# KyanChen/RSPrompter

Hardware: AMD Instinct MI355X
Metric: images/sec (1024x1024 synthetic tiles, rsprompter_anchor SAM-ViT-H, full predict path) (higher is better)
Workload: dtype f32 (fp32 in/out; GEMMs and attention as fp16x3 split-precision MFMA with fp32 accumulate); 1 GPU; rsprompter_anchor SAM-ViT-huge, batch 8x1024x1024 per GPU, 10 classes, seeded synthetic weights (the per-GPU slice of BASELINE.json configs[3] on 1 GPU); parallelism=single GPU

## Files before the change

### rsprompter_amd/csrc/t2i_fold.hip

```cpp
#include <type_traits>
#include "rsp_common.h"

namespace {

typedef __attribute__((address_space(3))) void* lptr_f;
typedef short v4s_f __attribute__((ext_vector_type(4)));

constexpr int FKT = 32, FNW = 3, FNT = FNW * 64, FNBUF = 2;
constexpr int FD = 256;
constexpr int FKCPR = 36, FPCPR = 17;
constexpr int FK_UNITS = FKT * FKCPR;
constexpr int FP_UNITS = 576;
constexpr int FTILE_UNITS = 2 * FK_UNITS + 2 * FP_UNITS;
constexpr int FNDMA = FTILE_UNITS / FNT;
constexpr int FBUF_BYTES = FTILE_UNITS * 16;
constexpr float F_PSCALE_LOG2 = 14.0f;
constexpr unsigned F_OOB = 0x80000000u;

static_assert(FK_UNITS % FNT == 0 && FP_UNITS % FNT == 0, "every DMA instruction reads one plane");

template <int I, int N, class F>
__device__ __forceinline__ void static_for_f(F&& f) {
  if constexpr (I < N) {
    f(std::integral_constant<int, I>{});
    static_for_f<I + 1, N>(f);
  }
}

__device__ __forceinline__ void split8_fast_f(const float* x, half8_t& hi, half8_t& lo) {
  float m1 = -1.0f;
  asm volatile("" : "+v"(m1));
#pragma unroll
  for (int i = 0; i < 8; i += 2) {
    const half2_t h2 = __builtin_bit_cast(half2_t, __builtin_amdgcn_cvt_pkrtz(x[i], x[i + 1]));
    const float r0 = __builtin_fmaf((float)h2[0], m1, x[i]), r1 = __builtin_fmaf((float)h2[1], m1, x[i + 1]);
    const half2_t l2 = __builtin_bit_cast(half2_t, __builtin_amdgcn_cvt_pkrtz(r0, r1));
    hi[i] = h2[0]; hi[i + 1] = h2[1]; lo[i] = l2[0]; lo[i + 1] = l2[1];
  }
}

struct T2iFoldP {
  const half_t* khi; const half_t* klo; int64_t k_rows;
  const half_t* phi; const half_t* plo;
  const half_t* qhi; const half_t* qlo; int64_t q_rows;
  const half_t* thi; const half_t* tlo;
  float* u;
  int N, ncols;
  float c_main, c_pe;
  float u_unscale;
};

template <int NPE>
__global__ __launch_bounds__(FNT) void sam_t2i_fold_kernel(const T2iFoldP p) {
  __shared__ __attribute__((aligned(1024))) unsigned char smem[FNBUF][FBUF_BYTES];
  __shared__ __attribute__((aligned(1024))) unsigned char sQl[FNW * 16 * 1024];
  const int tid = threadIdx.x, lane = tid & 63;
  const int wave = __builtin_amdgcn_readfirstlane(tid >> 6);
  const int hh = lane >> 5, l31 = lane & 31;
  const int r = blockIdx.x;
  const int N = p.N;
  const int nt = N / FKT;

  const __amdgpu_buffer_rsrc_t rKh = __builtin_amdgcn_make_buffer_rsrc(const_cast<half_t*>(p.khi), 0, (int)(p.k_rows * 512), 0x00020000);
  const __amdgpu_buffer_rsrc_t rKl = __builtin_amdgcn_make_buffer_rsrc(const_cast<half_t*>(p.klo), 0, (int)(p.k_rows * 512), 0x00020000);
  const __amdgpu_buffer_rsrc_t rPh = __builtin_amdgcn_make_buffer_rsrc(const_cast<half_t*>(p.phi), 0, N * 256, 0x00020000);
  const __amdgpu_buffer_rsrc_t rPl = __builtin_amdgcn_make_buffer_rsrc(const_cast<half_t*>(p.plo), 0, N * 256, 0x00020000);
  unsigned voff_k[6], voff_p[3];
#pragma unroll
  for (int i = 0; i < 6; ++i) {
    const int v = i * FNT + tid;
    const int row = v / FKCPR, pc = v - row * FKCPR;
    const int c = pc ^ ((row >> 2) & 3);
    voff_k[i] = pc < 32 ? (unsigned)(((int64_t)(c >> 2) * p.k_rows + row) * 64 + (c & 3) * 16) : F_OOB;
  }
#pragma unroll
  for (int i = 0; i < 3; ++i) {
    const int v = i * FNT + tid;
    const int row = v / FPCPR, pc = v - row * FPCPR;
    voff_p[i] = (row < FKT && pc < 16) ? (unsigned)(((int64_t)(pc >> 2) * N + row) * 64 + (pc & 3) * 16) : F_OOB;
  }
  const unsigned so_k0 = (unsigned)((int64_t)r * N * 64);
  const rsp_lds_addr_t smem_a = rsp_lds_addr((lptr_f)&smem[0][0]);
  auto issue_slot = [&](auto ic, int kt, int buf) {
    constexpr int i = decltype(ic)::value;
    const unsigned so_k = so_k0 + (unsigned)kt * (FKT * 64), so_p = (unsigned)kt * (FKT * 64);
    const rsp_lds_addr_t l = smem_a + buf * FBUF_BYTES + (i * FNT + wave * 64) * 16;
    const __amdgpu_buffer_rsrc_t rs = i < 6 ? rKh : (i < 12 ? rKl : (i < 15 ? rPh : rPl));
    const unsigned vo = i < 12 ? voff_k[i < 12 ? i % 6 : 0] : voff_p[i >= 12 ? (i - 12) % 3 : 0];
    const unsigned so = i < 12 ? so_k : so_p;
    RSP_BUFFER_LOAD_LDS_B128(rs, l, vo, so);
  };
  static_for_f<0, FNDMA>([&](auto ic) { issue_slot(ic, 0, 0); });

  const int64_t qrow = (int64_t)r * 96 + wave * 32 + l31;
  const int hb = NPE == 8 ? 0 : min((wave * 32) / (p.ncols >> 3), 8 - NPE);
  half8_t qh[16], th[NPE], tl[NPE];
  unsigned char* const my_ql = sQl + wave * (16 * 1024) + lane * 16;
#pragma unroll
  for (int st = 0; st < 16; ++st) {
    const int64_t o = ((int64_t)(st >> 1) * p.q_rows + qrow) * 32 + 16 * (st & 1) + 8 * hh;
    qh[st] = *reinterpret_cast<const half8_t*>(p.qhi + o);
    *reinterpret_cast<half8_t*>(my_ql + st * 1024) = *reinterpret_cast<const half8_t*>(p.qlo + o);
  }
#pragma unroll
  for (int s_ = 0; s_ < NPE; ++s_) {
    const int st = hb + s_;
    const int64_t o = ((int64_t)(st >> 1) * p.q_rows + qrow) * 32 + 16 * (st & 1) + 8 * hh;
    th[s_] = *reinterpret_cast<const half8_t*>(p.thi + o);
    tl[s_] = *reinterpret_cast<const half8_t*>(p.tlo + o);
  }

  f32x16 acc_o[8];
#pragma unroll
  for (int db = 0; db < 8; ++db)
#pragma unroll
    for (int e = 0; e < 16; ++e) acc_o[db][e] = 0.f;
  float m_run = -INFINITY, l_run = 0.f;

  const int k_row_off = l31 * (FKCPR * 16);
  const int k_swz = (l31 >> 2) & 3;
  const int p_row_off = l31 * (FPCPR * 16);
  const int li = lane & 15, g16 = (lane >> 4) & 1;
  const int v_row = 4 * hh + (li >> 2);
  const int v_c = 2 * g16 + ((li & 3) >> 1);
  const int v_b = 8 * (li & 1);

  for (int kt = 0; kt < nt; ++kt) {
    const int buf = kt & 1;
    asm volatile("s_waitcnt vmcnt(0)" ::: "memory");
    __builtin_amdgcn_s_barrier();
    const bool has_next = kt + 1 < nt;
    if (has_next) static_for_f<0, FNDMA>([&](auto ic) { issue_slot(ic, kt + 1, buf ^ 1); });
    const unsigned char* sb = &smem[buf][0];
    const unsigned char* sK0 = sb;
    const unsigned char* sK1 = sb + FK_UNITS * 16;
    const unsigned char* sP0 = sb + 2 * FK_UNITS * 16;
    const unsigned char* sP1 = sP0 + FP_UNITS * 16;

    f32x16 s0, s1, sp;
#pragma unroll
    for (int e = 0; e < 16; ++e) { s0[e] = 0.f; s1[e] = 0.f; sp[e] = 0.f; }
    {
      constexpr int LA = 1, NB = LA + 1;
      half8_t kfh[NB], kfl[NB];
      auto kread = [&](int st, half8_t& h8, half8_t& l8) {
        const int off = k_row_off + (((2 * st + hh) ^ k_swz) << 4);
        h8 = *reinterpret_cast<const half8_t*>(sK0 + off);
        l8 = *reinterpret_cast<const half8_t*>(sK1 + off);
      };
      auto pread = [&](int s_, half8_t& h8, half8_t& l8) {
        const int off = p_row_off + ((2 * (hb + s_) + hh) << 4);
        h8 = *reinterpret_cast<const half8_t*>(sP0 + off);
        l8 = *reinterpret_cast<const half8_t*>(sP1 + off);
      };
      half8_t qlf[NB];
      auto fetch = [&](auto jc) {
        constexpr int j = decltype(jc)::value, sl = j % NB;
        if constexpr (j < 16) {
          kread(j, kfh[sl], kfl[sl]);
          qlf[sl] = *reinterpret_cast<const half8_t*>(my_ql + j * 1024);
        } else if constexpr (j < 16 + NPE) pread(j - 16, kfh[sl], kfl[sl]);
      };
      static_for_f<0, LA>([&](auto jc) { fetch(jc); });
      static_for_f<0, 16 + NPE>([&](auto ic) {
        constexpr int i = decltype(ic)::value, cur = i % NB;
// ... 85 lines not shown
    for (int db = 0; db < 8; ++db)
#pragma unroll
      for (int g = 0; g < 4; ++g) {
        f32x4 o;
#pragma unroll
        for (int c = 0; c < 4; ++c) o[c] = acc_o[db][4 * g + c] * inv;
        *reinterpret_cast<f32x4*>(dst + db * 32 + 8 * g + 4 * hh) = o;
      }
  }
}

}

extern "C" int rsp_sam_t2i_fold(const uint16_t* keys_hi, const uint16_t* keys_lo, int64_t k_rows, int32_t keys_e,
                                const uint16_t* pek_hi, const uint16_t* pek_lo, int32_t pek_e, const uint16_t* qp_hi,
                                const uint16_t* qp_lo, int32_t qp_e, const uint16_t* tqx_hi, const uint16_t* tqx_lo,
                                int32_t tqx_e, int64_t q_rows, float* u, int32_t R, int32_t N, int32_t ncols,
                                rsp_stream_t stream) {
  if (!keys_hi || !keys_lo || !pek_hi || !pek_lo || !qp_hi || !qp_lo || !tqx_hi || !tqx_lo || !u || R < 0 || N <= 0 ||
      (N % FKT) || ncols <= 0 || ncols > 96 || (ncols & 7) || k_rows < (int64_t)R * N || q_rows < (int64_t)R * 96 ||
      k_rows * 512 > 0x7fffffffLL || (int64_t)N * 256 > 0x7fffffffLL)
    return RSP_EINVAL;
  if (R == 0) return RSP_OK;
  T2iFoldP p;
  p.khi = reinterpret_cast<const half_t*>(keys_hi); p.klo = reinterpret_cast<const half_t*>(keys_lo); p.k_rows = k_rows;
  p.phi = reinterpret_cast<const half_t*>(pek_hi); p.plo = reinterpret_cast<const half_t*>(pek_lo);
  p.qhi = reinterpret_cast<const half_t*>(qp_hi); p.qlo = reinterpret_cast<const half_t*>(qp_lo); p.q_rows = q_rows;
  p.thi = reinterpret_cast<const half_t*>(tqx_hi); p.tlo = reinterpret_cast<const half_t*>(tqx_lo);
  p.u = u; p.N = N; p.ncols = ncols;
  constexpr float LOG2E_F = 1.4426950408889634f;
  p.c_main = ldexpf(1.0f, -(keys_e + qp_e)) * LOG2E_F;
  p.c_pe = ldexpf(1.0f, -(pek_e + tqx_e)) * LOG2E_F;
  p.u_unscale = ldexpf(1.0f, -keys_e);
  const bool five = ncols >= 56;
  const dim3 g(R), b(FNT);
  hipStream_t s = (hipStream_t)stream;
  if (five) hipLaunchKernelGGL((sam_t2i_fold_kernel<5>), g, b, 0, s, p);
  else hipLaunchKernelGGL((sam_t2i_fold_kernel<8>), g, b, 0, s, p);
  RSP_CHECK_LAUNCH();
  return RSP_OK;
}
```

### rsprompter_amd/sam_decoder.py

```python
import math

import numpy as np
import torch

from . import ops
from .nnutil import HIPModule, add_param, infer_sam_arch, nchw_view, nhwc_view
from .registry import MODELS

HID = 256
HEADS = 8
MLP_DIM = 2048
N_MASK_TOKENS = 4


def _upscale2_k_order():
    return [32 * ((kp >> 4) >> 1) + 8 * ((8 * ((kp >> 4) & 1) + (kp & 7)) >> 2) + 4 * ((kp >> 3) & 1) + (kp & 3) for kp in range(64)]


def _add_linear(root, name, cout, cin):
    add_param(root, name + '.weight', (cout, cin))
    add_param(root, name + '.bias', (cout,))


def _add_ln(root, name, c):
# ... 13 lines not shown
    return root


HOOK_FORMS = ('accepted forms: attention_similarity 4-D [1 | B * Pb, 1, 1, N] (one bias row over the N image positions, shared '
              'or per prompt set; no per-head, per-token or other shape), with at most ops.SAM_T2I_MAX_TOKENS = 12 tokens; '
              'target_embedding [..., 256] that broadcasts to [B, Pb, 1, 256] (every other dimension 1 or equal)')


def persam_hooks(attention_similarity, target_embedding, B, Pb, N, T):
    R = B * Pb
    bias = te = None
    if attention_similarity is not None:
        a = attention_similarity
        if not torch.is_tensor(a) or a.dim() != 4 or a.shape[1] != 1 or a.shape[2] != 1 or a.shape[3] != N or \
                a.shape[0] not in (1, R):
            raise NotImplementedError(f'attention_similarity of shape {tuple(getattr(a, "shape", ()))} for B * Pb = {R}, N = {N}; '
                                      + HOOK_FORMS)
        if T > ops.SAM_T2I_MAX_TOKENS:
            raise NotImplementedError(f'attention_similarity with {T} tokens (the generic attention takes no bias); ' + HOOK_FORMS)
        bias = a.reshape(a.shape[0], N).to(torch.float32).contiguous()
    if target_embedding is not None:
        t = target_embedding
        ok = torch.is_tensor(t) and 1 <= t.dim() <= 4 and t.shape[-1] == HID
        if ok:
            b, pb, tk = ((1, 1, 1) + tuple(t.shape[:-1]))[-3:]
            ok = b in (1, B) and pb in (1, Pb) and tk == 1
        if not ok:
            raise NotImplementedError(f'target_embedding of shape {tuple(getattr(t, "shape", ()))} for B = {B}, Pb = {Pb}; '
                                      + HOOK_FORMS)
        t = t.to(torch.float32).reshape(b, pb, HID)
        te = t.reshape(1, HID) if b * pb == 1 else t.expand(B, Pb, HID).reshape(R, HID)
        te = te.contiguous()
    return bias, te


class SamMaskDecoderHIP(HIPModule):

    def __init__(self):
        super().__init__()
        add_param(self, 'iou_token.weight', (1, HID))
        add_param(self, 'mask_tokens.weight', (N_MASK_TOKENS, HID))
        for i in range(2):
            p = f'transformer.layers.{i}'
            _add_attn(self, p + '.self_attn', HID)
            _add_attn(self, p + '.cross_attn_token_to_image', HID // 2)
            _add_attn(self, p + '.cross_attn_image_to_token', HID // 2)
            for j in range(1, 5):
                _add_ln(self, f'{p}.layer_norm{j}', HID)
            _add_linear(self, p + '.mlp.lin1', MLP_DIM, HID)
            _add_linear(self, p + '.mlp.lin2', HID, MLP_DIM)
        _add_attn(self, 'transformer.final_attn_token_to_image', HID // 2)
        _add_ln(self, 'transformer.layer_norm_final_attn', HID)
        add_param(self, 'upscale_conv1.weight', (HID, HID // 4, 2, 2))
        add_param(self, 'upscale_conv1.bias', (HID // 4,))
        add_param(self, 'upscale_conv2.weight', (HID // 4, HID // 8, 2, 2))
        add_param(self, 'upscale_conv2.bias', (HID // 8,))
        _add_ln(self, 'upscale_layer_norm', HID // 4)
        for i in range(N_MASK_TOKENS):
            p = f'output_hypernetworks_mlps.{i}'
            _add_linear(self, p + '.proj_in', HID, HID)
            _add_linear(self, p + '.layers.0', HID, HID)
            _add_linear(self, p + '.proj_out', HID // 8, HID)
        _add_linear(self, 'iou_prediction_head.proj_in', HID, HID)
        _add_linear(self, 'iou_prediction_head.layers.0', HID, HID)
        _add_linear(self, 'iou_prediction_head.proj_out', N_MASK_TOKENS, HID)
        self._pe_cache = {}
# ... 50 lines not shown
                t[name] = ops.gemm(pe_rows, P[name])
            for pre, p in (('0.cross_attn_token_to_image', 'transformer.layers.0.cross_attn_token_to_image'),
                           ('1.cross_attn_token_to_image', 'transformer.layers.1.cross_attn_token_to_image'),
                           ('final', 'transformer.final_attn_token_to_image')):
                vb = _g(self, p + '.v_proj').bias
                t[pre + '.kv_proj'] = torch.cat([t[pre + '.k_proj'], vb.unsqueeze(0).expand(pe_rows.shape[0], -1)],
                                                1).contiguous()
                t[pre + '.pek_planes'] = ops.to_planes(t[pre + '.k_proj'])
            t['_table'] = pe_rows
            self._pe_cache = {key: t}
        return self._pe_cache[key]

    @staticmethod
    def _pe_key(pe_rows):
        return (pe_rows.data_ptr(), tuple(pe_rows.shape), pe_rows._version)

    def _ln(self, x, name, eps=1e-6, planes=False):
        m = _g(self, name)
        return ops.layernorm(x, m.weight, m.bias, eps, planes=planes)

    def _t2i(self, tq, kv, ao, R, T, N, kv_map=None, bias=None):
        d2, dh2 = HID // 2, (HID // 2) // HEADS
        if bias is not None:
            if T > ops.SAM_T2I_MAX_TOKENS:
                raise NotImplementedError(f'attention_similarity with {T} tokens; ' + HOOK_FORMS)
            return ops.sam_t2i_attention_bias(tq, kv, bias, ao, R=R, T=T, N=N, scale=dh2 ** -0.5, kv_map=kv_map)
        if T <= ops.SAM_T2I_MAX_TOKENS:
            return ops.sam_t2i_attention(tq, kv, ao, R=R, T=T, N=N, scale=dh2 ** -0.5, kv_map=kv_map)
        kvs = (N * 2 * d2, 2 * d2, dh2)
        return ops.attention(tq, kv, kv[:, d2:], ao, B=R, nh=HEADS, dh=dh2, Tq=T, Tk=N, scale=dh2 ** -0.5,
                             q_strides=(T * d2, d2, dh2), k_strides=kvs, v_strides=kvs,
                             o_strides=(T * d2, d2, dh2), kv_batch_map=kv_map)

    def _t2i_folded(self, pre, tq, keys_pl, pe_t, R, T, N):
        P = self._packed
        dh2 = (HID // 2) // HEADS
        tqx = ops.sam_fold_expand(tq, R, T, dh2 ** -0.5)
        qp = ops.gemm(tqx, P[pre + '.k_projT'], bias=None, out_planes=True, out_f32=False)
        u = ops.sam_t2i_fold(keys_pl, pe_t[pre + '.pek_planes'], qp, tqx, R=R, N=N, ncols=HEADS * T)
        full = ops.gemm(u, P[pre + '.v_proj'])
        return ops.sam_fold_gather(full, R, T)

    def _i2t(self, qi, kt, vt, ai, R, T, N, q_map=None):
        d2, dh2 = HID // 2, (HID // 2) // HEADS
        if T <= ops.SAM_I2T_MAX_TOKENS:
            return ops.sam_i2t_attention(qi, kt, vt, R=R, T=T, N=N, scale=dh2 ** -0.5, q_map=q_map, out_planes=ai)
        return ops.attention(qi, kt, vt, None, B=R, nh=HEADS, dh=dh2, Tq=N, Tk=T, scale=dh2 ** -0.5,
                             q_strides=(N * d2, d2, dh2), k_strides=(T * d2, d2, dh2), v_strides=(T * d2, d2, dh2),
                             o_strides=(N * d2, d2, dh2), q_batch_map=q_map, out_planes=ai)

    def _token_attn(self, q_in, k_in, v_in, pfx, R, T, res=None):
        P = self._packed
        q = ops.gemm(q_in, P[pfx + '.q_proj'])
        k = ops.gemm(k_in, P[pfx + '.k_proj'])
        v = ops.gemm(v_in, P[pfx + '.v_proj'])
        dh = HID // HEADS
        o = torch.empty_like(q)
        st = (T * HID, HID, dh)
        ops.attention(q, k, v, o, B=R, nh=HEADS, dh=dh, Tq=T, Tk=T, scale=dh ** -0.5,
                      q_strides=st, k_strides=st, v_strides=st, o_strides=st)
        return ops.gemm(o, P[pfx + '.out_proj'], res=res)

    def decode(self, image_embeddings, image_pe, sparse, dense_vec, roi_img, want_iou=True, src_rows=None, hw=None,
               multimask_output=False, src_is_identity=False, attn_bias=None, target_rows=None, **head_kw):
        R = sparse.shape[0]
        if src_rows is None:
            N = image_embeddings.shape[-2] * image_embeddings.shape[-1]
        else:
            N = hw[0] * hw[1]
# ... 96 lines not shown
        q = self._token_attn(qpe, qpe, q, '1.self_attn', R, T, res=q)
        q = self._ln(q, 'transformer.layers.1.layer_norm1')
        qpe = ops.add_rows(q, tokens0)
        tq = ops.gemm(qpe, P['1.cross_attn_token_to_image.q_proj'])
        fold = self.t2i_fold and T <= ops.SAM_T2I_FOLD_MAX_TOKENS and N % 32 == 0 and R * N * 512 < 2 ** 31
        kv = None
        if fold and attn_bias is None:
            ao = self._t2i_folded('1.cross_attn_token_to_image', tq, keys_pl, pe_t, R, T, N)
        else:
            kv = ops.gemm(keys_pl, P['1.cross_attn_token_to_image.kv_proj'], bias=None,
                          res=pe_t['1.cross_attn_token_to_image.kv_proj'], res_mod=N)
            self._t2i(tq, kv, ao, R, T, N, bias=attn_bias)
        q = ops.gemm(ao, P['1.cross_attn_token_to_image.out_proj'], res=q)
        q = self._ln(q, 'transformer.layers.1.layer_norm2')
        hmid = ops.gemm(q, P['1.lin1'], act=ops.ACT_RELU)
        q = ops.gemm(hmid, P['1.lin2'], res=q)
        q = self._ln(q, 'transformer.layers.1.layer_norm3')
        qpe = ops.add_rows(q, tokens0)
        qi = ops.gemm(keys_pl, P['1.cross_attn_image_to_token.q_proj'], bias=None,
                      res=pe_t['1.cross_attn_image_to_token.q_proj'], res_mod=N)
        kt = ops.gemm(qpe, P['1.cross_attn_image_to_token.k_proj'])
        vt = ops.gemm(q, P['1.cross_attn_image_to_token.v_proj'])
        m4 = _g(self, 'transformer.layers.1.layer_norm4')
        if fused:
            op = _g(self, 'transformer.layers.1.cross_attn_image_to_token.out_proj')
            keys_pl = ops.sam_i2t_fused(qi, kt, vt, op.weight.detach(), op.bias.detach(), m4.weight, m4.bias, R=R, T=T,
                                        N=N, scale=dh2 ** -0.5, eps=1e-6, res_planes=keys_pl)
        else:
            self._i2t(qi, kt, vt, ai, R, T, N)
            keys = ops.gemm(ai, P['1.cross_attn_image_to_token.out_proj'], res=keys_pl)
            keys_pl = ops.layernorm(keys, m4.weight, m4.bias, 1e-6, planes=True, f32=False)
            del keys

        qpe = ops.add_rows(q, tokens0)
        tq = ops.gemm(qpe, P['final.q_proj'])
        if fold:
            ao = self._t2i_folded('final', tq, keys_pl, pe_t, R, T, N)
        else:
            kv = ops.gemm(keys_pl, P['final.kv_proj'], bias=None, res=pe_t['final.kv_proj'], res_mod=N, out=kv)
            self._t2i(tq, kv, ao, R, T, N)
        q = ops.gemm(ao, P['final.out_proj'], res=q)
        q = self._ln(q, 'transformer.layer_norm_final_attn', eps=1e-5)
        del kv, qi, ai
        q3 = q.view(R, T, HID)
        stages = dict(keys=keys_pl, tokens=q3, up=None, hyper=[]) if self.keep_stages else None
        hold = [keys_pl]
        del keys_pl
        return self._heads(q3, hold, R, h, w, multimask_output, want_iou, stages, roi_img, src, **head_kw)

    def _output_tokens(self):
        return torch.cat([self.iou_token.weight, self.mask_tokens.weight], 0)

    def _hyper(self, q3, i, name=None):
        P = self._packed
        name = name or f'hyper{i}'
        mt = q3[:, 1 + i, :].contiguous()
        hy = ops.gemm(mt, P[name + '.proj_in'], act=ops.ACT_RELU)
        hy = ops.gemm(hy, P[name + '.layers.0'], act=ops.ACT_RELU)
        return ops.gemm(hy, P[name + '.proj_out'])

    def _iou_head(self, q3):
        P = self._packed
        it = q3[:, 0, :].contiguous()
        io = ops.gemm(it, P['iou.proj_in'], act=ops.ACT_RELU)
        io = ops.gemm(io, P['iou.layers.0'], act=ops.ACT_RELU)
        return ops.gemm(io, P['iou.proj_out'])

    def _heads(self, q3, hold, R, h, w, multimask_output, want_iou, stages, roi_img, src):
        P = self._packed
        keys_pl = hold.pop()

        toks = (1, 2, 3) if multimask_output else (0,)
        fused_up = self.upscale_fused and len(toks) == 1
        if not fused_up:
            up = ops.conv_transpose2x2(keys_pl.view(R, h, w, HID), *P['up1'], act=ops.ACT_GELU,
                                       ln=(self.upscale_layer_norm.weight, self.upscale_layer_norm.bias, 1e-6))
            del keys_pl
            if stages is not None:
                stages['up'] = up
        outs = []
        for i in toks:
            hy = self._hyper(q3, i)
            if stages is not None:
                stages['hyper'].append(hy)
            if fused_up:
                outs.append(ops.sam_upscale_fused(keys_pl, P['up1'][0], P['up1'][1], self.upscale_layer_norm.weight,
                                                  self.upscale_layer_norm.bias, 1e-6, P['up2p'][0], P['up2p'][1], hy,
                                                  h, w).view(R, 1, 4 * h, 4 * w))
                continue
            outs.append(ops.conv_transpose2x2(up, *P['up2'], act=ops.ACT_GELU, hyper=hy).view(R, 1, 4 * h, 4 * w))
        masks = outs[0] if len(outs) == 1 else torch.cat(outs, 1)
        self._last_stages = stages
        iou = None
        if want_iou:
            io = self._iou_head(q3)
            iou = io[:, 1:4].contiguous() if multimask_output else io[:, 0:1]
        return masks, iou

    def forward(self, image_embeddings, image_positional_embeddings, sparse_prompt_embeddings,
                dense_prompt_embeddings, multimask_output=False, attention_similarity=None,
                target_embedding=None, output_attentions=None, **head_kw):
        B = image_embeddings.shape[0]
        if sparse_prompt_embeddings.dim() == 4:
            Pb = sparse_prompt_embeddings.shape[1]
            sparse = sparse_prompt_embeddings.reshape(B * Pb, sparse_prompt_embeddings.shape[2], HID)
        else:
            Pb = 1
            sparse = sparse_prompt_embeddings
        bias, te = persam_hooks(attention_similarity, target_embedding, B, Pb,
                                image_embeddings.shape[-2] * image_embeddings.shape[-1], self.n_output_tokens + sparse.shape[1])
        dev = image_embeddings.device
        roi_img = torch.arange(B, dtype=torch.int32, device=dev)
        if Pb > 1:
            roi_img = roi_img.repeat_interleave(Pb)
        d = nhwc_view(dense_prompt_embeddings)
        if d.shape[0] not in (1, B):
            raise ValueError(f'dense_prompt_embeddings: batch {d.shape[0]} for {B} image embeddings')
        const = bool((d == d[:1, :1, :1]).all())
        if const:
            masks, iou = self.decode(image_embeddings, image_positional_embeddings, sparse.contiguous(),
                                     d[0, 0, 0].contiguous(), roi_img, multimask_output=bool(multimask_output),
                                     attn_bias=bias, target_rows=te, **head_kw)
        else:
            emb = nhwc_view(image_embeddings)
            _, h, w, C = emb.shape
            src = ops.add_rows(emb.reshape(B * h * w, C).contiguous(), d.reshape(-1, C).contiguous())
            masks, iou = self.decode(None, image_positional_embeddings, sparse.contiguous(), None, roi_img,
                                     src_rows=src, hw=(h, w), multimask_output=bool(multimask_output), attn_bias=bias,
# ... 43 lines not shown
            P[key] = convt_weights4(m.weight, m.bias)
        P['hq_w1'], P['hq_wf'] = hq_conv_weights(self.mask_conv1.weight, self.mask_conv2.weight)

    def _output_tokens(self):
        return torch.cat([self.iou_token.weight, self.mask_tokens.weight, self.hq_token.weight], 0)

    @torch.no_grad()
    def hq_features(self, image_embeddings, vit_features=None):
        if self._packed is None:
            self._pack()
        P = self._packed
        self.hq_feature_calls += 1
        emb = nhwc_view(image_embeddings)
        B, h, w, _ = emb.shape
        e = ops.conv_transpose2x2(emb, *P['enc1'], act=ops.ACT_GELU, ln=(self.encoder_norm.weight, self.encoder_norm.bias, 1e-6))
        f = ops.conv_transpose2x2(e, *P['enc2'])
        if vit_features is not None:
            if tuple(vit_features.shape) != (B, h, w, self.vit_dim):
                raise ValueError(f'intermediate embedding: expected [{B}, {h}, {w}, {self.vit_dim}], got {tuple(vit_features.shape)}')
            c = ops.conv_transpose2x2(vit_features.to(torch.float32).contiguous(), *P['vit1'])
            c = ops.layernorm(c.view(B * 4 * h * w, HID), self.compress_vit_norm.weight, self.compress_vit_norm.bias, 1e-6,
                              act=ops.ACT_GELU, planes=True, f32=False)
            c = ops.conv_transpose2x2(c.view(B, 2 * h, 2 * w, HID), *P['vit2'])
            f = ops.add_rows(f.view(-1, HID // 8), c.view(-1, HID // 8)).view(B, 4 * h, 4 * w, HID // 8)
        return f

    def decode(self, *args, hq_features=None, hq_token_only=False, src_is_identity=False, **kw):
        if hq_features is None:
            raise ValueError('SamHQMaskDecoderHIP.decode needs hq_features (see hq_features())')
        if src_is_identity:
            raise NotImplementedError('SamHQMaskDecoderHIP.decode: src_is_identity (one source per prompt set) is not taken')
        return super().decode(*args, hq_features=hq_features, hq_token_only=bool(hq_token_only), **kw)

    def _heads(self, q3, hold, R, h, w, multimask_output, want_iou, stages, roi_img, src, hq_features=None, hq_token_only=False):
        P = self._packed
        hold.pop()
        feat, hq_only = hq_features, hq_token_only
        if h != w:
            raise NotImplementedError(f'SamHQMaskDecoderHIP: a {h} x {w} embedding grid (HQ:999 is a spatial transpose only '
                                      'for a square grid)')
        if tuple(feat.shape[1:]) != (4 * h, 4 * w, HID // 8):
            raise ValueError(f'hq_features: expected [*, {4 * h}, {4 * w}, {HID // 8}], got {tuple(feat.shape)}')
        S = src.shape[0] // (h * w)
        src_t = src.view(S, h, w, HID).transpose(1, 2).contiguous()
        up = ops.conv_transpose2x2(src_t, *P['up1'], act=ops.ACT_GELU,
                                   ln=(self.upscale_layer_norm.weight, self.upscale_layer_norm.bias, 1e-6))
        io = self._iou_head(q3)
        hy_hq = self._hyper(q3, N_MASK_TOKENS, 'hq')
        if multimask_output:
            iou, order = torch.sort(io[:, 1:4], dim=1, descending=True, stable=True)
            hy = torch.stack([self._hyper(q3, i) for i in (1, 2, 3)], 1)
            hy = torch.gather(hy, 1, order.unsqueeze(-1).expand(-1, -1, hy.shape[-1])).contiguous()
        else:
            iou = io[:, 0:1]
            hy = self._hyper(q3, 0).unsqueeze(1).contiguous()
        if stages is not None:
            stages.update(up=up, hyper_hq=hy_hq, hyper=[hy[:, j] for j in range(hy.shape[1])])
        self._last_stages = stages
        rmap = roi_img.to(torch.int32).contiguous()
        res = ops.sam_hq_mask(up, P['up2'][0], P['up2'][1], P['hq_w1'], self.mask_conv1.bias, self.mask_norm.weight,
                              self.mask_norm.bias, 1e-6, P['hq_wf'], self.mask_conv2.bias, hy_hq, feat.contiguous(), rmap,
                              up_map=rmap, hyper_sam=None if hq_only else hy)
        masks = res.view(R, 1, 4 * h, 4 * w) if hq_only else res[1]
        return masks, (iou if want_iou else None)

    def forward(self, image_embeddings, image_positional_embeddings, sparse_prompt_embeddings, dense_prompt_embeddings,
                multimask_output=False, hq_token_only=False, intermediate_embeddings=None, attention_similarity=None,
                target_embedding=None, hq_features=None):
        if hq_features is None:
            vit = intermediate_embeddings[0] if intermediate_embeddings is not None and len(intermediate_embeddings) > 0 else None
            hq_features = self.hq_features(image_embeddings, vit)
        return super().forward(image_embeddings, image_positional_embeddings, sparse_prompt_embeddings,
                               dense_prompt_embeddings, multimask_output=multimask_output,
                               attention_similarity=attention_similarity, target_embedding=target_embedding,
                               hq_features=hq_features, hq_token_only=bool(hq_token_only))


@MODELS.register_module()
class RSSamMaskDecoder(HIPModule):
    def __init__(self, hf_pretrain_name, extra_config=None, init_cfg=None):
        super().__init__()
        self.mask_decoder = SamMaskDecoderHIP()

    def forward(self, *args, **kwargs):
        return self.mask_decoder(*args, **kwargs)


def image_wide_table(G, size):
# ... 71 lines not shown
```

Baseline: 51.84 images/s.

## Compute final token-to-image attention only for tokens the heads consume

The final decoder attention step now picks out only the output tokens the mask/IoU heads actually read (e.g. IoU plus one mask token when multimask is off). It runs the final q-projection, folded attention, out-projection and layernorm on that subset, and the heads index into it through a position map. The fold kernel gains a column-block variant that splits the head dimension across four waves and reduces scores through LDS, used when the column count is small; the old kernel stays for larger counts. This cuts per-prompt work in the last transformer stage, at the cost of extra gather copies and a cross-wave LDS reduction with an added barrier.

```diff
diff --git a/rsprompter_amd/csrc/t2i_fold.hip b/rsprompter_amd/csrc/t2i_fold.hip
--- a/rsprompter_amd/csrc/t2i_fold.hip
+++ b/rsprompter_amd/csrc/t2i_fold.hip
@@ -6,18 +6,20 @@
 typedef __attribute__((address_space(3))) void* lptr_f;
 typedef short v4s_f __attribute__((ext_vector_type(4)));
 
-constexpr int FKT = 32, FNW = 3, FNT = FNW * 64, FNBUF = 2;
+constexpr int FKT = 32, FNW = 4, FNT = FNW * 64, FNBUF = 2;
 constexpr int FD = 256;
 constexpr int FKCPR = 36, FPCPR = 17;
 constexpr int FK_UNITS = FKT * FKCPR;
 constexpr int FP_UNITS = 576;
 constexpr int FTILE_UNITS = 2 * FK_UNITS + 2 * FP_UNITS;
-constexpr int FNDMA = FTILE_UNITS / FNT;
+constexpr int FK_WI = FK_UNITS / 64, FP_WI = FP_UNITS / 64;
+constexpr int FTILE_WI = FTILE_UNITS / 64;
+constexpr int FNDMA = (FTILE_WI + FNW - 1) / FNW;
 constexpr int FBUF_BYTES = FTILE_UNITS * 16;
 constexpr float F_PSCALE_LOG2 = 14.0f;
 constexpr unsigned F_OOB = 0x80000000u;
 
-static_assert(FK_UNITS % FNT == 0 && FP_UNITS % FNT == 0, "every DMA instruction reads one plane");
+static_assert(FK_UNITS % 64 == 0 && FP_UNITS % 64 == 0, "every DMA instruction reads one plane");
 
 template <int I, int N, class F>
 __device__ __forceinline__ void static_for_f(F&& f) {
@@ -50,10 +52,10 @@
   float u_unscale;
 };
 
-template <int NPE>
+template <int NCB>
 __global__ __launch_bounds__(FNT) void sam_t2i_fold_kernel(const T2iFoldP p) {
   __shared__ __attribute__((aligned(1024))) unsigned char smem[FNBUF][FBUF_BYTES];
-  __shared__ __attribute__((aligned(1024))) unsigned char sQl[FNW * 16 * 1024];
+  __shared__ __attribute__((aligned(1024))) unsigned char sX[FNW * NCB * 4 * 1024];
   const int tid = threadIdx.x, lane = tid & 63;
   const int wave = __builtin_amdgcn_readfirstlane(tid >> 6);
   const int hh = lane >> 5, l31 = lane & 31;
@@ -61,61 +63,81 @@
   const int N = p.N;
   const int nt = N / FKT;
 
+  unsigned voff[FNDMA];
+#pragma unroll
+  for (int i = 0; i < FNDMA; ++i) {
+    const int j = i * FNW + wave;
+    const bool is_k = j < 2 * FK_WI;
+    const int jp = is_k ? (j < FK_WI ? j : j - FK_WI) : (j - 2 * FK_WI < FP_WI ? j - 2 * FK_WI : j - 2 * FK_WI - FP_WI);
+    const int v = jp * 64 + lane;
+    const int krow = v / FKCPR, kpc = v - krow * FKCPR;
+    const int c = kpc ^ ((krow >> 2) & 3);
+    const unsigned vk = kpc < 32 ? (unsigned)(((int64_t)(c >> 2) * p.k_rows + krow) * 64 + (c & 3) * 16) : F_OOB;
+    const int prow = v / FPCPR, ppc = v - prow * FPCPR;
+    const unsigned vp = (prow < FKT && ppc < 16) ? (unsigned)(((int64_t)(ppc >> 2) * N + prow) * 64 + (ppc & 3) * 16) : F_OOB;
+    voff[i] = is_k ? vk : vp;
+  }
+  const unsigned so_k0 = (unsigned)((int64_t)r * N * 64);
+  const rsp_lds_addr_t smem_a = rsp_lds_addr((lptr_f)&smem[0][0]);
   const __amdgpu_buffer_rsrc_t rKh = __builtin_amdgcn_make_buffer_rsrc(const_cast<half_t*>(p.khi), 0, (int)(p.k_rows * 512), 0x00020000);
   const __amdgpu_buffer_rsrc_t rKl = __builtin_amdgcn_make_buffer_rsrc(const_cast<half_t*>(p.klo), 0, (int)(p.k_rows * 512), 0x00020000);
   const __amdgpu_buffer_rsrc_t rPh = __builtin_amdgcn_make_buffer_rsrc(const_cast<half_t*>(p.phi), 0, N * 256, 0x00020000);
   const __amdgpu_buffer_rsrc_t rPl = __builtin_amdgcn_make_buffer_rsrc(const_cast<half_t*>(p.plo), 0, N * 256, 0x00020000);
-  unsigned voff_k[6], voff_p[3];
-#pragma unroll
-  for (int i = 0; i < 6; ++i) {
-    const int v = i * FNT + tid;
-    const int row = v / FKCPR, pc = v - row * FKCPR;
-    const int c = pc ^ ((row >> 2) & 3);
-    voff_k[i] = pc < 32 ? (unsigned)(((int64_t)(c >> 2) * p.k_rows + row) * 64 + (c & 3) * 16) : F_OOB;
-  }
-#pragma unroll
-  for (int i = 0; i < 3; ++i) {
-    const int v = i * FNT + tid;
-    const int row = v / FPCPR, pc = v - row * FPCPR;
-    voff_p[i] = (row < FKT && pc < 16) ? (unsigned)(((int64_t)(pc >> 2) * N + row) * 64 + (pc & 3) * 16) : F_OOB;
-  }
-  const unsigned so_k0 = (unsigned)((int64_t)r * N * 64);
-  const rsp_lds_addr_t smem_a = rsp_lds_addr((lptr_f)&smem[0][0]);
   auto issue_slot = [&](auto ic, int kt, int buf) {
     constexpr int i = decltype(ic)::value;
-    const unsigned so_k = so_k0 + (unsigned)kt * (FKT * 64), so_p = (unsigned)kt * (FKT * 64);
-    const rsp_lds_addr_t l = smem_a + buf * FBUF_BYTES + (i * FNT + wave * 64) * 16;
-    const __amdgpu_buffer_rsrc_t rs = i < 6 ? rKh : (i < 12 ? rKl : (i < 15 ? rPh : rPl));
-    const unsigned vo = i < 12 ? voff_k[i < 12 ? i % 6 : 0] : voff_p[i >= 12 ? (i - 12) % 3 : 0];
-    const unsigned so = i < 12 ? so_k : so_p;
-    RSP_BUFFER_LOAD_LDS_B128(rs, l, vo, so);
+    constexpr auto plane_of = [](int j) { return j < FK_WI ? 0 : (j < 2 * FK_WI ? 1 : (j < 2 * FK_WI + FP_WI ? 2 : 3)); };
+    constexpr int pl0 = plane_of(i * FNW), pl1 = plane_of(i * FNW + FNW - 1 < FTILE_WI ? i * FNW + FNW - 1 : FTILE_WI - 1);
+    constexpr int edge = pl0 == 0 ? FK_WI : (pl0 == 1 ? 2 * FK_WI : 2 * FK_WI + FP_WI);
+    const bool second = pl0 != pl1 && i * FNW + wave >= edge;
+    const __amdgpu_buffer_rsrc_t rs = pl0 == 0 ? (second ? rKl : rKh) : (pl0 == 1 ? (second ? rPh : rKl) : (pl0 == 2 ? (second ? rPl : rPh) : rPl));
+    const bool is_k = pl0 == 0 || (pl0 == 1 && !second);
+    const unsigned so = (is_k ? so_k0 : 0u) + (unsigned)kt * (FKT * 64);
+    const rsp_lds_addr_t l = smem_a + buf * FBUF_BYTES + (i * FNW + wave) * 1024;
+    const unsigned vo = voff[i];
+    if (i * FNW + FNW - 1 < FTILE_WI || i * FNW + wave < FTILE_WI) RSP_BUFFER_LOAD_LDS_B128(rs, l, vo, so);
   };
   static_for_f<0, FNDMA>([&](auto ic) { issue_slot(ic, 0, 0); });
 
-  const int64_t qrow = (int64_t)r * 96 + wave * 32 + l31;
-  const int hb = NPE == 8 ? 0 : min((wave * 32) / (p.ncols >> 3), 8 - NPE);
-  half8_t qh[16], th[NPE], tl[NPE];
-  unsigned char* const my_ql = sQl + wave * (16 * 1024) + lane * 16;
-#pragma unroll
-  for (int st = 0; st < 16; ++st) {
-    const int64_t o = ((int64_t)(st >> 1) * p.q_rows + qrow) * 32 + 16 * (st & 1) + 8 * hh;
-    qh[st] = *reinterpret_cast<const half8_t*>(p.qhi + o);
-    *reinterpret_cast<half8_t*>(my_ql + st * 1024) = *reinterpret_cast<const half8_t*>(p.qlo + o);
-  }
-#pragma unroll
-  for (int s_ = 0; s_ < NPE; ++s_) {
-    const int st = hb + s_;
-    const int64_t o = ((int64_t)(st >> 1) * p.q_rows + qrow) * 32 + 16 * (st & 1) + 8 * hh;
-    th[s_] = *reinterpret_cast<const half8_t*>(p.thi + o);
-    tl[s_] = *reinterpret_cast<const half8_t*>(p.tlo + o);
-  }
-
-  f32x16 acc_o[8];
-#pragma unroll
-  for (int db = 0; db < 8; ++db)
-#pragma unroll
-    for (int e = 0; e < 16; ++e) acc_o[db][e] = 0.f;
-  float m_run = -INFINITY, l_run = 0.f;
+  half8_t qh[NCB][4], ql[NCB][4], th[NCB][2], tl[NCB][2];
+#pragma unroll
+  for (int cb = 0; cb < NCB; ++cb) {
+    const int64_t qrow = (int64_t)r * 96 + cb * 32 + l31;
+#pragma unroll
+    for (int j = 0; j < 4; ++j) {
+      const int st = 4 * wave + j;
+      const int64_t o = ((int64_t)(st >> 1) * p.q_rows + qrow) * 32 + 16 * (st & 1) + 8 * hh;
+      qh[cb][j] = *reinterpret_cast<const half8_t*>(p.qhi + o);
+      ql[cb][j] = *reinterpret_cast<const half8_t*>(p.qlo + o);
+    }
+#pragma unroll
+    for (int jh = 0; jh < 2; ++jh) {
+      const int st = wave + 4 * jh;
+      const int64_t o = ((int64_t)(st >> 1) * p.q_rows + qrow) * 32 + 16 * (st & 1) + 8 * hh;
+      th[cb][jh] = *reinterpret_cast<const half8_t*>(p.thi + o);
+      tl[cb][jh] = *reinterpret_cast<const half8_t*>(p.tlo + o);
+    }
+  }
+#pragma unroll
+  for (int cb = 0; cb < NCB; ++cb) {
+#pragma unroll
+    for (int j = 0; j < 4; ++j) asm volatile("" : "+v"(qh[cb][j]), "+v"(ql[cb][j]));
+#pragma unroll
+    for (int jh = 0; jh < 2; ++jh) asm volatile("" : "+v"(th[cb][jh]), "+v"(tl[cb][jh]));
+  }
+  const int T = p.ncols >> 3;
+  auto head_in_block = [&](int h, int cb) { return h * T < 32 * (cb + 1) && (h + 1) * T > 32 * cb; };
+
+  f32x16 acc_o[NCB][2];
+  float m_run[NCB], l_run[NCB];
+#pragma unroll
+  for (int cb = 0; cb < NCB; ++cb) {
+#pragma unroll
+    for (int jd = 0; jd < 2; ++jd)
+#pragma unroll
+      for (int e = 0; e < 16; ++e) acc_o[cb][jd][e] = 0.f;
+    m_run[cb] = -INFINITY;
+    l_run[cb] = 0.f;
+  }
 
   const int k_row_off = l31 * (FKCPR * 16);
   const int k_swz = (l31 >> 2) & 3;
@@ -124,6 +146,7 @@
   const int v_row = 4 * hh + (li >> 2);
   const int v_c = 2 * g16 + ((li & 3) >> 1);
   const int v_b = 8 * (li & 1);
+  unsigned char* const my_x = sX + wave * (NCB * 4 * 1024) + lane * 16;
 
   for (int kt = 0; kt < nt; ++kt) {
     const int buf = kt & 1;
@@ -131,6 +154,228 @@
     __builtin_amdgcn_s_barrier();
     const bool has_next = kt + 1 < nt;
     if (has_next) static_for_f<0, FNDMA>([&](auto ic) { issue_slot(ic, kt + 1, buf ^ 1); });
+    const unsigned char* sb = &smem[buf][0];
+    const unsigned char* sK0 = sb;
+    const unsigned char* sK1 = sb + FK_UNITS * 16;
+    const unsigned char* sP0 = sb + 2 * FK_UNITS * 16;
+    const unsigned char* sP1 = sP0 + FP_UNITS * 16;
+
+    {
+      half8_t kfh[4], kfl[4], pfh[2], pfl[2];
+#pragma unroll
+      for (int j = 0; j < 4; ++j) {
+        const int off = k_row_off + (((2 * (4 * wave + j) + hh) ^ k_swz) << 4);
+        kfh[j] = *reinterpret_cast<const half8_t*>(sK0 + off);
+        kfl[j] = *reinterpret_cast<const half8_t*>(sK1 + off);
+      }
+#pragma unroll
+      for (int jh = 0; jh < 2; ++jh) {
+        const int off = p_row_off + ((2 * (wave + 4 * jh) + hh) << 4);
+        pfh[jh] = *reinterpret_cast<const half8_t*>(sP0 + off);
+        pfl[jh] = *reinterpret_cast<const half8_t*>(sP1 + off);
+      }
+#pragma unroll
+      for (int cb = 0; cb < NCB; ++cb) {
+        f32x16 s, sp;
+#pragma unroll
+        for (int e = 0; e < 16; ++e) { s[e] = 0.f; sp[e] = 0.f; }
+#pragma unroll
+        for (int j = 0; j < 4; ++j) {
+          s = __builtin_amdgcn_mfma_f32_32x32x16_f16(kfl[j], qh[cb][j], s, 0, 0, 0);
+          s = __builtin_amdgcn_mfma_f32_32x32x16_f16(kfh[j], ql[cb][j], s, 0, 0, 0);
+          s = __builtin_amdgcn_mfma_f32_32x32x16_f16(kfh[j], qh[cb][j], s, 0, 0, 0);
+        }
+#pragma unroll
+        for (int jh = 0; jh < 2; ++jh)
+          if (head_in_block(wave + 4 * jh, cb)) {
+            sp = __builtin_amdgcn_mfma_f32_32x32x16_f16(pfl[jh], th[cb][jh], sp, 0, 0, 0);
+            sp = __builtin_amdgcn_mfma_f32_32x32x16_f16(pfh[jh], tl[cb][jh], sp, 0, 0, 0);
+            sp = __builtin_amdgcn_mfma_f32_32x32x16_f16(pfh[jh], th[cb][jh], sp, 0, 0, 0);
+          }
+#pragma unroll
+        for (int g = 0; g < 4; ++g) {
+          f32x4 o;
+#pragma unroll
+          for (int c = 0; c < 4; ++c) o[c] = fmaf(s[4 * g + c], p.c_main, sp[4 * g + c] * p.c_pe);
+          *reinterpret_cast<f32x4*>(my_x + (cb * 4 + g) * 1024) = o;
+        }
+      }
+    }
+    asm volatile("s_waitcnt lgkmcnt(0)" ::: "memory");
+    __builtin_amdgcn_s_barrier();
+
+    typedef __attribute__((address_space(3))) v4s_f* lv4;
+    v4s_f va[2][2][4];
+#pragma unroll
+    for (int s_ = 0; s_ < 2; ++s_)
+#pragma unroll
+      for (int jd = 0; jd < 2; ++jd) {
+        const int row0 = 16 * s_ + v_row;
+        const int c = 4 * (2 * wave + jd) + v_c;
+        const int a0 = row0 * (FKCPR * 16) + ((c ^ hh) << 4) + v_b;
+        const int a1 = (row0 + 8) * (FKCPR * 16) + ((c ^ ((hh + 2) & 3)) << 4) + v_b;
+        va[s_][jd][0] = __builtin_amdgcn_ds_read_tr16_b64_v4i16((lv4)(sK0 + a0));
+        va[s_][jd][1] = __builtin_amdgcn_ds_read_tr16_b64_v4i16((lv4)(sK0 + a1));
+        va[s_][jd][2] = __builtin_amdgcn_ds_read_tr16_b64_v4i16((lv4)(sK1 + a0));
+        va[s_][jd][3] = __builtin_amdgcn_ds_read_tr16_b64_v4i16((lv4)(sK1 + a1));
+      }
+
+#pragma unroll
+    for (int cb = 0; cb < NCB; ++cb) {
+      float sc[16];
+#pragma unroll
+      for (int g = 0; g < 4; ++g) {
+        const unsigned char* x = sX + (cb * 4 + g) * 1024 + lane * 16;
+        f32x4 a = *reinterpret_cast<const f32x4*>(x);
+#pragma unroll
+        for (int w = 1; w < FNW; ++w) {
+          const f32x4 b = *reinterpret_cast<const f32x4*>(x + w * (NCB * 4 * 1024));
+#pragma unroll
+          for (int c = 0; c < 4; ++c) a[c] += b[c];
+        }
+#pragma unroll
+        for (int c = 0; c < 4; ++c) sc[4 * g + c] = a[c];
+      }
+      float tmax = -INFINITY;
+#pragma unroll
+      for (int e = 0; e < 16; ++e) tmax = fmaxf(tmax, sc[e]);
+      tmax = fmaxf(tmax, __shfl_xor(tmax, 32, 64));
+      const float m_new = fmaxf(m_run[cb], tmax);
+      const float alpha = __builtin_amdgcn_exp2f(m_run[cb] - m_new);
+      const float kk = F_PSCALE_LOG2 - m_new;
+      float psum = 0.f;
+#pragma unroll
+      for (int e = 0; e < 16; ++e) {
+        sc[e] = __builtin_amdgcn_exp2f(sc[e] + kk);
+        psum += sc[e];
+      }
+      l_run[cb] = l_run[cb] * alpha + psum;
+      m_run[cb] = m_new;
+      if (__builtin_amdgcn_ballot_w64(alpha != 1.0f) != 0) {
+#pragma unroll
+        for (int jd = 0; jd < 2; ++jd)
+#pragma unroll
+          for (int e = 0; e < 16; ++e) acc_o[cb][jd][e] *= alpha;
+      }
+#pragma unroll
+      for (int s_ = 0; s_ < 2; ++s_) {
+        half8_t ph, pl;
+        split8_fast_f(sc + 8 * s_, ph, pl);
+#pragma unroll
+        for (int jd = 0; jd < 2; ++jd) {
+          union { v4s_f s4[2]; half8_t h8; } uh, ul;
+          uh.s4[0] = va[s_][jd][0]; uh.s4[1] = va[s_][jd][1]; ul.s4[0] = va[s_][jd][2]; ul.s4[1] = va[s_][jd][3];
+          acc_o[cb][jd] = __builtin_amdgcn_mfma_f32_32x32x16_f16(ul.h8, ph, acc_o[cb][jd], 0, 0, 0);
+          acc_o[cb][jd] = __builtin_amdgcn_mfma_f32_32x32x16_f16(uh.h8, pl, acc_o[cb][jd], 0, 0, 0);
+          acc_o[cb][jd] = __builtin_amdgcn_mfma_f32_32x32x16_f16(uh.h8, ph, acc_o[cb][jd], 0, 0, 0);
+        }
+      }
+    }
+  }
+
+#pragma unroll
+  for (int cb = 0; cb < NCB; ++cb) {
+    const float l_tot = l_run[cb] + __shfl_xor(l_run[cb], 32, 64);
+    const int col = cb * 32 + l31;
+    if (col < p.ncols) {
+      const float inv = p.u_unscale / l_tot;
+      float* dst = p.u + ((int64_t)r * 96 + col) * FD + wave * 64;
+#pragma unroll
+      for (int jd = 0; jd < 2; ++jd)
+#pragma unroll
+        for (int g = 0; g < 4; ++g) {
+          f32x4 o;
+#pragma unroll
+          for (int c = 0; c < 4; ++c) o[c] = acc_o[cb][jd][4 * g + c] * inv;
+          *reinterpret_cast<f32x4*>(dst + jd * 32 + 8 * g + 4 * hh) = o;
+        }
+    }
+  }
+}
+
+constexpr int CNW = 3, CNT = CNW * 64, CNDMA = FTILE_UNITS / CNT, NPE = 5;
+static_assert(FK_UNITS % CNT == 0 && FP_UNITS % CNT == 0, "every DMA instruction reads one plane");
+
+__global__ __launch_bounds__(CNT) void sam_t2i_fold_cols_kernel(const T2iFoldP p) {
+  __shared__ __attribute__((aligned(1024))) unsigned char smem[FNBUF][FBUF_BYTES];
+  __shared__ __attribute__((aligned(1024))) unsigned char sQl[CNW * 16 * 1024];
+  const int tid = threadIdx.x, lane = tid & 63;
+  const int wave = __builtin_amdgcn_readfirstlane(tid >> 6);
+  const int hh = lane >> 5, l31 = lane & 31;
+  const int r = blockIdx.x;
+  const int N = p.N;
+  const int nt = N / FKT;
+
+  const __amdgpu_buffer_rsrc_t rKh = __builtin_amdgcn_make_buffer_rsrc(const_cast<half_t*>(p.khi), 0, (int)(p.k_rows * 512), 0x00020000);
+  const __amdgpu_buffer_rsrc_t rKl = __builtin_amdgcn_make_buffer_rsrc(const_cast<half_t*>(p.klo), 0, (int)(p.k_rows * 512), 0x00020000);
+  const __amdgpu_buffer_rsrc_t rPh = __builtin_amdgcn_make_buffer_rsrc(const_cast<half_t*>(p.phi), 0, N * 256, 0x00020000);
+  const __amdgpu_buffer_rsrc_t rPl = __builtin_amdgcn_make_buffer_rsrc(const_cast<half_t*>(p.plo), 0, N * 256, 0x00020000);
+  unsigned voff_k[6], voff_p[3];
+#pragma unroll
+  for (int i = 0; i < 6; ++i) {
+    const int v = i * CNT + tid;
+    const int row = v / FKCPR, pc = v - row * FKCPR;
+    const int c = pc ^ ((row >> 2) & 3);
+    voff_k[i] = pc < 32 ? (unsigned)(((int64_t)(c >> 2) * p.k_rows + row) * 64 + (c & 3) * 16) : F_OOB;
+  }
+#pragma unroll
+  for (int i = 0; i < 3; ++i) {
+    const int v = i * CNT + tid;
+    const int row = v / FPCPR, pc = v - row * FPCPR;
+    voff_p[i] = (row < FKT && pc < 16) ? (unsigned)(((int64_t)(pc >> 2) * N + row) * 64 + (pc & 3) * 16) : F_OOB;
+  }
+  const unsigned so_k0 = (unsigned)((int64_t)r * N * 64);
+  const rsp_lds_addr_t smem_a = rsp_lds_addr((lptr_f)&smem[0][0]);
+  auto issue_slot = [&](auto ic, int kt, int buf) {
+    constexpr int i = decltype(ic)::value;
+    const unsigned so_k = so_k0 + (unsigned)kt * (FKT * 64), so_p = (unsigned)kt * (FKT * 64);
+    const rsp_lds_addr_t l = smem_a + buf * FBUF_BYTES + (i * CNT + wave * 64) * 16;
+    const __amdgpu_buffer_rsrc_t rs = i < 6 ? rKh : (i < 12 ? rKl : (i < 15 ? rPh : rPl));
+    const unsigned vo = i < 12 ? voff_k[i < 12 ? i % 6 : 0] : voff_p[i >= 12 ? (i - 12) % 3 : 0];
+    const unsigned so = i < 12 ? so_k : so_p;
+    RSP_BUFFER_LOAD_LDS_B128(rs, l, vo, so);
+  };
+  static_for_f<0, CNDMA>([&](auto ic) { issue_slot(ic, 0, 0); });
+
+  const int64_t qrow = (int64_t)r * 96 + wave * 32 + l31;
+  const int hb = min((wave * 32) / (p.ncols >> 3), 8 - NPE);
+  half8_t qh[16], th[NPE], tl[NPE];
+  unsigned char* const my_ql = sQl + wave * (16 * 1024) + lane * 16;
+#pragma unroll
+  for (int st = 0; st < 16; ++st) {
+    const int64_t o = ((int64_t)(st >> 1) * p.q_rows + qrow) * 32 + 16 * (st & 1) + 8 * hh;
+    qh[st] = *reinterpret_cast<const half8_t*>(p.qhi + o);
+    *reinterpret_cast<half8_t*>(my_ql + st * 1024) = *reinterpret_cast<const half8_t*>(p.qlo + o);
+  }
+#pragma unroll
+  for (int s_ = 0; s_ < NPE; ++s_) {
+    const int st = hb + s_;
+    const int64_t o = ((int64_t)(st >> 1) * p.q_rows + qrow) * 32 + 16 * (st & 1) + 8 * hh;
+    th[s_] = *reinterpret_cast<const half8_t*>(p.thi + o);
+    tl[s_] = *reinterpret_cast<const half8_t*>(p.tlo + o);
+  }
+
+  f32x16 acc_o[8];
+#pragma unroll
+  for (int db = 0; db < 8; ++db)
+#pragma unroll
+    for (int e = 0; e < 16; ++e) acc_o[db][e] = 0.f;
+  float m_run = -INFINITY, l_run = 0.f;
+
+  const int k_row_off = l31 * (FKCPR * 16);
+  const int k_swz = (l31 >> 2) & 3;
+  const int p_row_off = l31 * (FPCPR * 16);
+  const int li = lane & 15, g16 = (lane >> 4) & 1;
+  const int v_row = 4 * hh + (li >> 2);
+  const int v_c = 2 * g16 + ((li & 3) >> 1);
+  const int v_b = 8 * (li & 1);
+
+  for (int kt = 0; kt < nt; ++kt) {
+    const int buf = kt & 1;
+    asm volatile("s_waitcnt vmcnt(0)" ::: "memory");
+    __builtin_amdgcn_s_barrier();
+    const bool has_next = kt + 1 < nt;
+    if (has_next) static_for_f<0, CNDMA>([&](auto ic) { issue_slot(ic, kt + 1, buf ^ 1); });
     const unsigned char* sb = &smem[buf][0];
     const unsigned char* sK0 = sb;
     const unsigned char* sK1 = sb + FK_UNITS * 16;
@@ -282,11 +527,11 @@
   p.c_main = ldexpf(1.0f, -(keys_e + qp_e)) * LOG2E_F;
   p.c_pe = ldexpf(1.0f, -(pek_e + tqx_e)) * LOG2E_F;
   p.u_unscale = ldexpf(1.0f, -keys_e);
-  const bool five = ncols >= 56;
   const dim3 g(R), b(FNT);
   hipStream_t s = (hipStream_t)stream;
-  if (five) hipLaunchKernelGGL((sam_t2i_fold_kernel<5>), g, b, 0, s, p);
-  else hipLaunchKernelGGL((sam_t2i_fold_kernel<8>), g, b, 0, s, p);
+  if (ncols <= 32) hipLaunchKernelGGL((sam_t2i_fold_kernel<1>), g, b, 0, s, p);
+  else if (ncols <= 64) hipLaunchKernelGGL((sam_t2i_fold_kernel<2>), g, b, 0, s, p);
+  else hipLaunchKernelGGL(sam_t2i_fold_cols_kernel, g, dim3(CNT), 0, s, p);
   RSP_CHECK_LAUNCH();
   return RSP_OK;
 }
diff --git a/rsprompter_amd/sam_decoder.py b/rsprompter_amd/sam_decoder.py
--- a/rsprompter_amd/sam_decoder.py
+++ b/rsprompter_amd/sam_decoder.py
@@ -69,6 +69,11 @@
         te = t.reshape(1, HID) if b * pb == 1 else t.expand(B, Pb, HID).reshape(R, HID)
         te = te.contiguous()
     return bias, te
+
+
+def _take_tokens(x, R, T, tokens):
+    x3 = x.view(R, T, x.shape[-1])
+    return torch.stack([x3[:, t] for t in tokens], 1).reshape(R * len(tokens), x.shape[-1])
 
 
 class SamMaskDecoderHIP(HIPModule):
@@ -185,9 +190,12 @@
                              q_strides=(T * d2, d2, dh2), k_strides=kvs, v_strides=kvs,
                              o_strides=(T * d2, d2, dh2), kv_batch_map=kv_map)
 
-    def _t2i_folded(self, pre, tq, keys_pl, pe_t, R, T, N):
+    def _t2i_folded(self, pre, tq, keys_pl, pe_t, R, T, N, tokens=None):
         P = self._packed
         dh2 = (HID // 2) // HEADS
+        if tokens is not None:
+            tq = _take_tokens(tq, R, T, tokens)
+            T = len(tokens)
         tqx = ops.sam_fold_expand(tq, R, T, dh2 ** -0.5)
         qp = ops.gemm(tqx, P[pre + '.k_projT'], bias=None, out_planes=True, out_f32=False)
         u = ops.sam_t2i_fold(keys_pl, pe_t[pre + '.pek_planes'], qp, tqx, R=R, N=N, ncols=HEADS * T)
@@ -350,41 +358,56 @@
             keys_pl = ops.layernorm(keys, m4.weight, m4.bias, 1e-6, planes=True, f32=False)
             del keys
 
-        qpe = ops.add_rows(q, tokens0)
+        sel = None if (self.keep_stages or not fold) else self._final_tokens(multimask_output, want_iou, **head_kw)
+        tok_pos = None
+        Tf = T
+        if sel is not None and len(sel) < T:
+            tok_pos = {t: k for k, t in enumerate(sel)}
+            Tf = len(sel)
+            q = _take_tokens(q, R, T, sel)
+            qpe = ops.add_rows(q, _take_tokens(tokens0, R, T, sel))
+        else:
+            qpe = ops.add_rows(q, tokens0)
         tq = ops.gemm(qpe, P['final.q_proj'])
         if fold:
-            ao = self._t2i_folded('final', tq, keys_pl, pe_t, R, T, N)
+            ao = self._t2i_folded('final', tq, keys_pl, pe_t, R, Tf, N)
         else:
             kv = ops.gemm(keys_pl, P['final.kv_proj'], bias=None, res=pe_t['final.kv_proj'], res_mod=N, out=kv)
             self._t2i(tq, kv, ao, R, T, N)
         q = ops.gemm(ao, P['final.out_proj'], res=q)
         q = self._ln(q, 'transformer.layer_norm_final_attn', eps=1e-5)
         del kv, qi, ai
-        q3 = q.view(R, T, HID)
+        q3 = q.view(R, Tf, HID)
         stages = dict(keys=keys_pl, tokens=q3, up=None, hyper=[]) if self.keep_stages else None
         hold = [keys_pl]
         del keys_pl
+        if tok_pos is not None:
+            head_kw = dict(head_kw, tok_pos=tok_pos)
         return self._heads(q3, hold, R, h, w, multimask_output, want_iou, stages, roi_img, src, **head_kw)
 
     def _output_tokens(self):
         return torch.cat([self.iou_token.weight, self.mask_tokens.weight], 0)
 
-    def _hyper(self, q3, i, name=None):
+    def _final_tokens(self, multimask_output, want_iou, **head_kw):
+        toks = (1, 2, 3) if multimask_output else (0,)
+        return ((0,) if want_iou else ()) + tuple(1 + i for i in toks)
+
+    def _hyper(self, q3, i, name=None, tok_pos=None):
         P = self._packed
         name = name or f'hyper{i}'
-        mt = q3[:, 1 + i, :].contiguous()
+        mt = q3[:, 1 + i if tok_pos is None else tok_pos[1 + i], :].contiguous()
         hy = ops.gemm(mt, P[name + '.proj_in'], act=ops.ACT_RELU)
         hy = ops.gemm(hy, P[name + '.layers.0'], act=ops.ACT_RELU)
         return ops.gemm(hy, P[name + '.proj_out'])
 
-    def _iou_head(self, q3):
-        P = self._packed
-        it = q3[:, 0, :].contiguous()
+    def _iou_head(self, q3, tok_pos=None):
+        P = self._packed
+        it = q3[:, 0 if tok_pos is None else tok_pos[0], :].contiguous()
         io = ops.gemm(it, P['iou.proj_in'], act=ops.ACT_RELU)
         io = ops.gemm(io, P['iou.layers.0'], act=ops.ACT_RELU)
         return ops.gemm(io, P['iou.proj_out'])
 
-    def _heads(self, q3, hold, R, h, w, multimask_output, want_iou, stages, roi_img, src):
+    def _heads(self, q3, hold, R, h, w, multimask_output, want_iou, stages, roi_img, src, tok_pos=None):
         P = self._packed
         keys_pl = hold.pop()
 
@@ -398,7 +421,7 @@
                 stages['up'] = up
         outs = []
         for i in toks:
-            hy = self._hyper(q3, i)
+            hy = self._hyper(q3, i, tok_pos=tok_pos)
             if stages is not None:
                 stages['hyper'].append(hy)
             if fused_up:
@@ -411,7 +434,7 @@
         self._last_stages = stages
         iou = None
         if want_iou:
-            io = self._iou_head(q3)
+            io = self._iou_head(q3, tok_pos)
             iou = io[:, 1:4].contiguous() if multimask_output else io[:, 0:1]
         return masks, iou
 
@@ -521,7 +544,11 @@
             raise NotImplementedError('SamHQMaskDecoderHIP.decode: src_is_identity (one source per prompt set) is not taken')
         return super().decode(*args, hq_features=hq_features, hq_token_only=bool(hq_token_only), **kw)
 
-    def _heads(self, q3, hold, R, h, w, multimask_output, want_iou, stages, roi_img, src, hq_features=None, hq_token_only=False):
+    def _final_tokens(self, multimask_output, want_iou, **head_kw):
+        return (0,) + ((2, 3, 4) if multimask_output else (1,)) + (1 + N_MASK_TOKENS,)
+
+    def _heads(self, q3, hold, R, h, w, multimask_output, want_iou, stages, roi_img, src, hq_features=None, hq_token_only=False,
+               tok_pos=None):
         P = self._packed
         hold.pop()
         feat, hq_only = hq_features, hq_token_only
@@ -534,15 +561,15 @@
         src_t = src.view(S, h, w, HID).transpose(1, 2).contiguous()
         up = ops.conv_transpose2x2(src_t, *P['up1'], act=ops.ACT_GELU,
                                    ln=(self.upscale_layer_norm.weight, self.upscale_layer_norm.bias, 1e-6))
-        io = self._iou_head(q3)
-        hy_hq = self._hyper(q3, N_MASK_TOKENS, 'hq')
+        io = self._iou_head(q3, tok_pos)
+        hy_hq = self._hyper(q3, N_MASK_TOKENS, 'hq', tok_pos)
         if multimask_output:
             iou, order = torch.sort(io[:, 1:4], dim=1, descending=True, stable=True)
-            hy = torch.stack([self._hyper(q3, i) for i in (1, 2, 3)], 1)
+            hy = torch.stack([self._hyper(q3, i, tok_pos=tok_pos) for i in (1, 2, 3)], 1)
             hy = torch.gather(hy, 1, order.unsqueeze(-1).expand(-1, -1, hy.shape[-1])).contiguous()
         else:
             iou = io[:, 0:1]
-            hy = self._hyper(q3, 0).unsqueeze(1).contiguous()
+            hy = self._hyper(q3, 0, tok_pos=tok_pos).unsqueeze(1).contiguous()
         if stages is not None:
             stages.update(up=up, hyper_hq=hy_hq, hyper=[hy[:, j] for j in range(hy.shape[1])])
         self._last_stages = stages
```

Result: no change. 52.07 images/s, median of 6 (+0.4%).
